# reazon-research/ReazonSpeech

Measured on AMD Instinct MI355X. Metric: RTFx (audio-sec/wall-sec), FastConformer-RNNT 619M batch=256, higher is better.
Workload: dtype bf16

## Files before the change

### reazonspeech_amd/csrc/k_frontend.hip

```cpp
#include "rs_common.h"

namespace {

constexpr int NFFT = 512;
constexpr int NBIN = 257;
constexpr int FB_MAXW = 32;
constexpr int WAVES = 4;
constexpr int FRAMES_PER_WAVE = 4;
constexpr int MAX_HOP = 256;
constexpr int SPAN_MAX = (WAVES * FRAMES_PER_WAVE - 1) * MAX_HOP + NFFT;

struct FrontParams {
    const float* audio; const int32_t* lens; float* raw; int32_t* n_frames;
    const float* window;
    const float* twiddle;
    const int32_t* fb_idx;
    const float* fb_w;
    int audio_stride, pad_left, pad_right, t_max, n_mels, win_length, hop;
    float preemph, log_guard;
    int kind;
};

__device__ __forceinline__ float fetch_sample(const float* __restrict__ a, int i, int pad_left, int len) {
    const int j = i - pad_left;
    return (j >= 0 && j < len) ? a[j] : 0.0f;
}

__device__ __forceinline__ float2 cmul(float2 a, float2 w) { return make_float2(a.x * w.x - a.y * w.y, a.x * w.y + a.y * w.x); }

__device__ __forceinline__ void dft8(float2 (&a)[8]) {
    constexpr float S = 0.70710678118654752f;
    float2 b[8];
#pragma unroll
    for (int j = 0; j < 4; ++j) {
        b[j] = make_float2(a[j].x + a[j + 4].x, a[j].y + a[j + 4].y);
        b[j + 4] = make_float2(a[j].x - a[j + 4].x, a[j].y - a[j + 4].y);
    }
    b[5] = make_float2(S * (b[5].x + b[5].y), S * (b[5].y - b[5].x));
    b[6] = make_float2(b[6].y, -b[6].x);
    b[7] = make_float2(S * (b[7].y - b[7].x), -S * (b[7].x + b[7].y));
    float2 c[8];
#pragma unroll
    for (int h = 0; h < 8; h += 4) {
        c[h + 0] = make_float2(b[h].x + b[h + 2].x, b[h].y + b[h + 2].y);
        c[h + 2] = make_float2(b[h].x - b[h + 2].x, b[h].y - b[h + 2].y);
        c[h + 1] = make_float2(b[h + 1].x + b[h + 3].x, b[h + 1].y + b[h + 3].y);
        const float2 d = make_float2(b[h + 1].x - b[h + 3].x, b[h + 1].y - b[h + 3].y);
        c[h + 3] = make_float2(d.y, -d.x);
    }
    a[0] = make_float2(c[0].x + c[1].x, c[0].y + c[1].y); a[4] = make_float2(c[0].x - c[1].x, c[0].y - c[1].y);
    a[2] = make_float2(c[2].x + c[3].x, c[2].y + c[3].y); a[6] = make_float2(c[2].x - c[3].x, c[2].y - c[3].y);
    a[1] = make_float2(c[4].x + c[5].x, c[4].y + c[5].y); a[5] = make_float2(c[4].x - c[5].x, c[4].y - c[5].y);
    a[3] = make_float2(c[6].x + c[7].x, c[6].y + c[7].y); a[7] = make_float2(c[6].x - c[7].x, c[6].y - c[7].y);
}

__global__ __launch_bounds__(64 * WAVES) void logmel_kernel(FrontParams p) {
    __shared__ float2 buf[WAVES][8 * 68];
    __shared__ float pw[WAVES][2][NBIN + 3];
    __shared__ float2 tw[NFFT / 2];
    __shared__ float ys[SPAN_MAX];
    __shared__ float win_s[NFFT];
    const int lane = threadIdx.x & 63, wave = threadIdx.x >> 6;
    const int b = blockIdx.y;
    const int len = p.lens[b];
    const int Lp = len + p.pad_left + p.pad_right;
    const int n_valid = p.kind == 2 ? (Lp + p.hop / 2) / p.hop
                                    : Lp / p.hop + (p.kind == 1 ? 1 : 0);
    if (blockIdx.x == 0 && threadIdx.x == 0) p.n_frames[b] = n_valid;
    const float* a = p.audio + (size_t)b * p.audio_stride;
    if ((int)blockIdx.x * WAVES * FRAMES_PER_WAVE >= min(n_valid, p.t_max)) return;
    tw[threadIdx.x] = reinterpret_cast<const float2*>(p.twiddle)[threadIdx.x];
    const int centre_off = (NFFT - p.win_length) / 2;
    const int f0 = blockIdx.x * WAVES * FRAMES_PER_WAVE;
    const int i_base = p.kind == 2 ? f0 * p.hop + p.hop / 2 - p.win_length / 2 : f0 * p.hop - NFFT / 2 + centre_off;
    const int span = (WAVES * FRAMES_PER_WAVE - 1) * p.hop + NFFT;
    for (int idx = threadIdx.x; idx < span; idx += blockDim.x) {
        int i = i_base + idx;
        float y = 0.0f;
        if (p.kind == 1 && Lp > 1) {
            i = i < 0 ? -i : i;
            i = i >= Lp ? 2 * (Lp - 1) - i : i;
            i = i < 0 ? 0 : i;
        }
        if (p.kind == 2 && Lp > 0) {
            for (int bounce = 0; bounce < 8 && (i < 0 || i >= Lp); ++bounce) i = i < 0 ? -i - 1 : 2 * Lp - 1 - i;
            i = i < 0 ? 0 : (i >= Lp ? Lp - 1 : i);
        }
        if (i >= 0 && i < Lp) {
            const float x0 = fetch_sample(a, i, p.pad_left, len);
            if (p.kind == 2) y = x0;
            else y = i >= 1 ? x0 - p.preemph * fetch_sample(a, i - 1, p.pad_left, len) : x0;
        }
        ys[idx] = y;
    }
    for (int idx = threadIdx.x; idx < NFFT; idx += blockDim.x) win_s[idx] = idx < p.win_length ? p.window[idx] : 0.0f;
    __syncthreads();
    const int frame_base = (blockIdx.x * WAVES + wave) * FRAMES_PER_WAVE;
    auto wave_sync = [&]() {
        __builtin_amdgcn_fence(__ATOMIC_ACQ_REL, "wavefront");
        __builtin_amdgcn_wave_barrier();
    };
    auto w512 = [&](int j) -> float2 {
        const float2 w = tw[j & 255];
        return (j & 256) ? make_float2(-w.x, -w.y) : w;
    };
    auto sample = [&](int t, int n) -> float {
        if (t >= n_valid || t >= p.t_max) return 0.0f;
        return ys[(t - f0) * p.hop + n] * win_s[n];
    };
    auto frame_mean = [&](int t) -> float {
        if (t >= n_valid || t >= p.t_max) return 0.0f;
        float sm = 0.0f;
        for (int n = lane; n < p.win_length; n += 64) sm += ys[(t - f0) * p.hop + n];
        return wave_sum(sm) / (float)p.win_length;
    };
    auto sample_kaldi = [&](int t, int n, float mean) -> float {
        if (t >= n_valid || t >= p.t_max || n >= p.win_length) return 0.0f;
        const float* fr = ys + (t - f0) * p.hop;
        const float cur = fr[n] - mean, prev = fr[n > 0 ? n - 1 : 0] - mean;
        return (cur - p.preemph * prev) * win_s[n];
    };
    const int k1 = lane & 7, hi = lane >> 3;

    for (int fi = 0; fi < FRAMES_PER_WAVE; fi += 2) {
        const int t = frame_base + fi;
        if (t >= n_valid || t >= p.t_max) break;
        float2* z = buf[wave];
        float2 v[8];
        if (p.kind == 2) {
            const float m0 = frame_mean(t), m1 = frame_mean(t + 1);
#pragma unroll
            for (int k = 0; k < 8; ++k) v[k] = make_float2(sample_kaldi(t, lane + 64 * k, m0), sample_kaldi(t + 1, lane + 64 * k, m1));
        } else {
#pragma unroll
            for (int k = 0; k < 8; ++k) v[k] = make_float2(sample(t, lane + 64 * k), sample(t + 1, lane + 64 * k));
        }
        dft8(v);
#pragma unroll
        for (int q = 0; q < 8; ++q) z[q * 68 + lane] = q ? cmul(v[q], w512(lane * q)) : v[q];
        wave_sync();
#pragma unroll
        for (int l1 = 0; l1 < 8; ++l1) v[l1] = z[k1 * 68 + hi + 8 * l1];
        wave_sync();
        dft8(v);
#pragma unroll
        for (int m1 = 0; m1 < 8; ++m1)
            z[m1 * 64 + ((hi * 8 + k1 + 8 * m1) & 63)] = m1 ? cmul(v[m1], w512(8 * hi * m1)) : v[m1];
        wave_sync();
#pragma unroll
        for (int l2 = 0; l2 < 8; ++l2) v[l2] = z[hi * 64 + ((l2 * 8 + k1 + 8 * hi) & 63)];
        wave_sync();
        dft8(v);
#pragma unroll
        for (int m2 = 0; m2 < 8; ++m2) z[lane + 64 * m2] = v[m2];
        wave_sync();
        for (int k = lane; k < NBIN; k += 64) {
            const float2 zk = z[k], zn = z[(NFFT - k) & (NFFT - 1)];
            const float ar = 0.5f * (zk.x + zn.x), ai = 0.5f * (zk.y - zn.y);
            const float br = 0.5f * (zk.y + zn.y), bi = 0.5f * (zn.x - zk.x);
            pw[wave][0][k] = ar * ar + ai * ai;
            pw[wave][1][k] = br * br + bi * bi;
        }
        wave_sync();
        for (int idx = lane; idx < 2 * p.n_mels; idx += 64) {
            const int f = idx >= p.n_mels, m = idx - f * p.n_mels;
            if (t + f < n_valid && t + f < p.t_max) {
                const int k0 = p.fb_idx[2 * m], cnt = p.fb_idx[2 * m + 1];
                const float* w = p.fb_w + m * FB_MAXW;
                float acc = 0.0f;
                for (int j = 0; j < cnt; ++j) acc = fmaf(w[j], pw[wave][f][k0 + j], acc);
                p.raw[((size_t)b * p.t_max + t + f) * p.n_mels + m] = p.kind >= 1 ? logf(fmaxf(acc, p.log_guard)) : logf(acc + p.log_guard);
            }
        }
        wave_sync();
    }
}

__global__ __launch_bounds__(1024) void feat_normalize_kernel(const float* __restrict__ raw,
                                                              const int32_t* __restrict__ n_frames, int t_max,
                                                              int n_mels, float eps, float* __restrict__ out) {
    __shared__ float4 red[1024];
    __shared__ float4 mean_s[32], rstd_s[32];
    const int b = blockIdx.x;
    const int n = min(n_frames[b], t_max);
    const int Q = n_mels >> 2;
    const int RG = 1000 / Q;
    const int tid = threadIdx.x;
    const int q = tid % Q, rg = tid / Q;
    const bool act = rg < RG;
    const float4* r4 = reinterpret_cast<const float4*>(raw + (size_t)b * t_max * n_mels);
    auto reduce_rows = [&](float4 v) -> float4 {
        red[tid] = act ? v : make_float4(0.f, 0.f, 0.f, 0.f);
        __syncthreads();
        float4 acc = make_float4(0.f, 0.f, 0.f, 0.f);
        if (tid < Q) {
            for (int g = 0; g < RG; ++g) {
                const float4 x = red[g * Q + tid];
                acc.x += x.x; acc.y += x.y; acc.z += x.z; acc.w += x.w;
            }
        }
        return acc;
    };
    float4 s = make_float4(0.f, 0.f, 0.f, 0.f);
    if (act)
#pragma unroll 8
        for (int t = rg; t < n; t += RG) {
            const float4 x = r4[(size_t)t * Q + q];
            s.x += x.x; s.y += x.y; s.z += x.z; s.w += x.w;
        }
    s = reduce_rows(s);
    if (tid < Q) {
        const float inv = 1.0f / (float)n;
        mean_s[tid] = make_float4(s.x * inv, s.y * inv, s.z * inv, s.w * inv);
    }
    __syncthreads();
    const float4 mean = mean_s[q];
    float4 m2 = make_float4(0.f, 0.f, 0.f, 0.f);
    if (act)
#pragma unroll 8
        for (int t = rg; t < n; t += RG) {
            const float4 x = r4[(size_t)t * Q + q];
            const float a = x.x - mean.x, bb = x.y - mean.y, c = x.z - mean.z, d = x.w - mean.w;
            m2.x += a * a; m2.y += bb * bb; m2.z += c * c; m2.w += d * d;
        }
    m2 = reduce_rows(m2);
    if (tid < Q) {
        const float dn = (float)(n - 1);
        rstd_s[tid] = n > 1 ? make_float4(1.0f / (sqrtf(m2.x / dn) + eps), 1.0f / (sqrtf(m2.y / dn) + eps),
                                          1.0f / (sqrtf(m2.z / dn) + eps), 1.0f / (sqrtf(m2.w / dn) + eps))
                            : make_float4(0.f, 0.f, 0.f, 0.f);
    }
    __syncthreads();
    const float4 rstd = rstd_s[q];
    float4* o4 = reinterpret_cast<float4*>(out + (size_t)b * t_max * n_mels);
    if (act)
#pragma unroll 8
        for (int t = rg; t < t_max; t += RG) {
            float4 y = make_float4(0.f, 0.f, 0.f, 0.f);
            if (t < n) {
                const float4 x = r4[(size_t)t * Q + q];
                y = make_float4((x.x - mean.x) * rstd.x, (x.y - mean.y) * rstd.y, (x.z - mean.z) * rstd.z,
                                (x.w - mean.w) * rstd.w);
            }
            o4[(size_t)t * Q + q] = y;
        }
}

__global__ __launch_bounds__(256) void feat_mvn_kernel(const float* __restrict__ raw, const int32_t* __restrict__ n_frames, int t_max,
                                                       int n_mels, const float* __restrict__ mean, const float* __restrict__ istd,
                                                       float* __restrict__ out) {
    const int b = blockIdx.y;
    const int i = blockIdx.x * 256 + threadIdx.x;
    if (i >= t_max * n_mels) return;
    const int t = i / n_mels, m = i - t * n_mels;
    const size_t at = (size_t)b * t_max * n_mels + i;
    out[at] = t < n_frames[b] ? (raw[at] - mean[m]) * istd[m] : 0.0f;
}

}

int rs_launch_frontend(rs_ctx* ctx, const float* audio, const int32_t* lens, int B, int audio_stride,
                       int pad_left, int pad_right, int t_max, float* feats, int32_t* n_frames, float* raw,
                       hipStream_t s) {
    const rs_dims& d = ctx->d;
    if (B <= 0 || t_max <= 0) return RS_OK;
    if (d.n_fft != NFFT) return rs_fail(ctx, RS_EINVAL, "frontend: only n_fft=512 is built");
    if (d.n_mels > 128 || d.n_mels % 4 || d.win_length > NFFT || d.hop_length < 1 || d.hop_length > MAX_HOP)
        return rs_fail(ctx, RS_EINVAL, "frontend: n_mels must be a multiple of 4 up to 128, win <= 512, hop <= %d", MAX_HOP);
    FrontParams p;
    p.audio = audio; p.lens = lens; p.raw = raw; p.n_frames = n_frames;
    p.window = ctx->fe_window; p.twiddle = ctx->fe_twiddle; p.fb_idx = ctx->fe_fb_idx; p.fb_w = ctx->fe_fb_w;
    p.audio_stride = audio_stride; p.pad_left = pad_left; p.pad_right = pad_right; p.t_max = t_max;
    p.n_mels = d.n_mels; p.win_length = d.win_length; p.hop = d.hop_length;
    p.preemph = d.preemph; p.log_guard = d.log_guard;
    p.kind = d.frontend_kind;
    const int fpb = WAVES * FRAMES_PER_WAVE;
    const dim3 grid((t_max + fpb - 1) / fpb, B), block(64 * WAVES);
    if (d.frontend_kind == 2) {
        p.raw = feats;
        RS_HIP(ctx, hipMemsetAsync(feats, 0, (size_t)B * t_max * d.n_mels * 4, s));
    }
    const double bytes = (double)B * ((double)t_max * d.hop_length * 4.0 + (double)t_max * d.n_mels * 4.0 * 3.0);
    rs_prof_begin(ctx, RS_PROF_FRONTEND, s, (double)B * t_max * (5.0 * 512 * 9 + 3 * 257 + 2 * 600), bytes);
    hipLaunchKernelGGL(logmel_kernel, grid, block, 0, s, p);
    if (d.frontend_kind == 2) {
    } else if (d.frontend_kind == 1)
        hipLaunchKernelGGL(feat_mvn_kernel, dim3((t_max * d.n_mels + 255) / 256, B), dim3(256), 0, s, raw, n_frames, t_max, d.n_mels,
                           ctx->fe_mvn_mean, ctx->fe_mvn_istd, feats);
    else
        hipLaunchKernelGGL(feat_normalize_kernel, dim3(B), dim3(1024), 0, s, raw, n_frames, t_max, d.n_mels, d.norm_eps,
                           feats);
    rs_prof_end(ctx, RS_PROF_FRONTEND, s);
    RS_CHECK_LAUNCH(ctx, "frontend");
    return RS_OK;
}
```

### reazonspeech_amd/csrc/rs_api.hip

```cpp
#include <stdarg.h>
#include <stdlib.h>
#include <string.h>

#include <mutex>
#include <set>
#include <utility>

#include "rs_common.h"

size_t rs_rnnt_workspace_bytes(const rs_ctx* ctx, int B);
size_t rs_rnnt_alsd_workspace_bytes_impl(const rs_ctx* ctx, int B, int beam, int cap);
size_t rs_rnnt_beam_workspace_bytes_impl(const rs_ctx* ctx, int B, int beam, int tp_max, int max_pops);
int rs_rnnt_beam_impl(rs_ctx* ctx, const float* joint_enc, const int32_t* enc_lens, int B, int tp_max, int beam, int score_norm,
                      int max_pops, int out_cap, int32_t* ids, int32_t* frames, int32_t* n_ids, float* scores, int32_t* pops,
                      void* workspace, size_t workspace_bytes, hipStream_t s);
int rs_rnnt_alsd_impl(rs_ctx* ctx, const float* joint_enc, const int32_t* enc_lens, int B, int tp_max, int beam, double ratio,
                      int abs_len, int score_norm, int merge, int out_cap, int32_t* ids, int32_t* steps, int32_t* n_ids,
                      float* scores, void* workspace, size_t workspace_bytes, hipStream_t s);
int rs_rnnt_greedy_impl(rs_ctx* ctx, const float* joint_enc, const int32_t* enc_lens, int B, int tp_max, int u_max,
                        int32_t* ids, int32_t* frames, int32_t* n_ids, void* workspace, size_t workspace_bytes,
                        hipStream_t s);

int rs_fail(rs_ctx* ctx, int code, const char* fmt, ...) {
    char buf[512];
// ... 157 lines not shown
    r.get("sub.out.b", dm, ctx->sub_out_b);
    ctx->layers.assign(d.n_layers, rs_layer_w{});
    for (int i = 0; i < d.n_layers; ++i) {
        rs_layer_w& L = ctx->layers[i];
        const std::string p = "L" + std::to_string(i) + ".";
        r.get(p + "ln_ff1.g", dm, L.ln_ff1_g); r.get(p + "ln_ff1.b", dm, L.ln_ff1_b);
        r.get(p + "ff1.w1", ff * dm, L.ff1_w1); r.get(p + "ff1.b1", ff, L.ff1_b1);
        r.get(p + "ff1.w2", dm * ff, L.ff1_w2); r.get(p + "ff1.b2", dm, L.ff1_b2);
        r.get(p + "ln_att.g", dm, L.ln_att_g); r.get(p + "ln_att.b", dm, L.ln_att_b);
        r.get(p + "att.qkv.w", 3 * dm * dm, L.qkv_w); r.get(p + "att.qkv.b", 3 * dm, L.qkv_b);
        r.get(p + "att.out.w", dm * dm, L.out_w); r.get(p + "att.out.b", dm, L.out_b);
        r.get(p + "att.pos.w", dm * dm, L.pos_w);
        r.get(p + "att.bias_u", dm, L.bias_u); r.get(p + "att.bias_v", dm, L.bias_v);
        r.get(p + "ln_conv.g", dm, L.ln_conv_g); r.get(p + "ln_conv.b", dm, L.ln_conv_b);
        r.get(p + "conv.pw1.w", 2 * dm * dm, L.pw1_w); r.get(p + "conv.pw1.b", 2 * dm, L.pw1_b);
        r.get(p + "conv.dw.w", (size_t)d.conv_kernel * dm, L.dw_w); r.get(p + "conv.dw.b", dm, L.dw_b);
        r.get(p + "conv.pw2.w", dm * dm, L.pw2_w); r.get(p + "conv.pw2.b", dm, L.pw2_b);
        r.get(p + "ln_ff2.g", dm, L.ln_ff2_g); r.get(p + "ln_ff2.b", dm, L.ln_ff2_b);
        r.get(p + "ff2.w1", ff * dm, L.ff2_w1); r.get(p + "ff2.b1", ff, L.ff2_b1);
        r.get(p + "ff2.w2", dm * ff, L.ff2_w2); r.get(p + "ff2.b2", dm, L.ff2_b2);
        r.get(p + "ln_out.g", dm, L.ln_out_g); r.get(p + "ln_out.b", dm, L.ln_out_b);
    }
    r.get("joint.enc.w", J * dm, ctx->jenc_w); r.get("joint.enc.b", J, ctx->jenc_b);
    r.get("pred.embed", V * H, ctx->embed);
    for (int l = 0; l < d.pred_layers; ++l) {
        const std::string p = "pred.lstm" + std::to_string(l);
        r.get(p + ".w", 4 * H * 2 * H, ctx->lstm_w[l]);
        r.get(p + ".b", 4 * H, ctx->lstm_b[l]);
    }
    r.get("joint.pred.w", J * H, ctx->jpred_w); r.get("joint.pred.b", J, ctx->jpred_b);
    r.get("joint.out.w", ((V + 15) / 16 * 16) * J, ctx->jout_w); r.get("joint.out.b", V, ctx->jout_b);
    if (r.rc != RS_OK) return r.rc;
    {
        const size_t Vpad = (V + 15) / 16 * 16;
        const bool any = ctx->tensors.count("joint.out.w16") || ctx->tensors.count("joint.out.wrm") ||
                         ctx->tensors.count("joint.out.bpad") || ctx->tensors.count("joint.out.wmax");
        ctx->jout_w16 = nullptr; ctx->jout_wrm = ctx->jout_bpad = ctx->jout_wmax = nullptr;
        if (any) {
            r.get("joint.out.w16", Vpad * J, ctx->jout_w16);
            r.get("joint.out.wrm", V * J, ctx->jout_wrm);
            r.get("joint.out.bpad", Vpad, ctx->jout_bpad);
            r.get("joint.out.wmax", (size_t)4, ctx->jout_wmax);
            if (r.rc != RS_OK) return r.rc;
        }
        for (int l = 0; l < d.pred_layers; ++l) {
            const std::string nm = "pred.lstm" + std::to_string(l) + ".w4";
            ctx->lstm_w4[l] = nullptr;
            if (ctx->tensors.count(nm)) { r.get(nm, 4 * H * 2 * H, ctx->lstm_w4[l]); if (r.rc != RS_OK) return r.rc; }
        }
        if (!ctx->env_read) {
            ctx->env_read = true;
            if (const char* e = getenv("RS_DECODE_SCREEN")) ctx->decode_screen = atoi(e) != 0;
            if (const char* nw = getenv("RS_DECODE_NARROW")) ctx->decode_narrow = atoi(nw) != 0;
            if (const char* fg = getenv("RS_FUSE_GLU")) ctx->fuse_glu = atoi(fg) != 0;
            if (const char* dn = getenv("RS_DEFER_OUT_NORM")) ctx->defer_out_norm = atoi(dn) != 0;
        }
    }
    ctx->has_f32 = false;
    if (ctx->tensors.count("sub.out.w.f32")) {
        rs_f32_weights& w = ctx->f32;
        for (int s = 1; s < d.sub_stages && d.sub_kind == 0; ++s) r.get("sub.pw" + std::to_string(s) + ".w.f32", C * C, w.sub_pw_w[s - 1]);
        if (d.sub_kind == 1) r.get("sub.conv1.w.f32", C * 9 * C, w.sub_conv1_w);
        if (d.ctc_vocab > 0) r.get("ctc.w.f32", (size_t)rs_ctc_pad(d.ctc_vocab) * dm, w.ctc_w);
        r.get("sub.out.w.f32", dm * C * ctx->sub_freq, w.sub_out_w);
        w.layers.assign(d.n_layers, rs_layer_w32{});
        for (int i = 0; i < d.n_layers; ++i) {
            rs_layer_w32& L = w.layers[i];
            const std::string p = "L" + std::to_string(i) + ".";
            r.get(p + "ff1.w1.f32", ff * dm, L.ff1_w1); r.get(p + "ff1.w2.f32", dm * ff, L.ff1_w2);
            r.get(p + "ff2.w1.f32", ff * dm, L.ff2_w1); r.get(p + "ff2.w2.f32", dm * ff, L.ff2_w2);
            r.get(p + "att.qkv.w.f32", 3 * dm * dm, L.qkv_w); r.get(p + "att.out.w.f32", dm * dm, L.out_w);
            r.get(p + "att.pos.w.f32", dm * dm, L.pos_w);
            r.get(p + "conv.pw1.w.f32", 2 * dm * dm, L.pw1_w); r.get(p + "conv.pw1.b.f32", 2 * dm, L.pw1_b);
            r.get(p + "conv.pw2.w.f32", dm * dm, L.pw2_w);
        }
        r.get("joint.enc.w.f32", J * dm, w.jenc_w);
        if (r.rc != RS_OK) return r.rc;
        auto pt = ctx->tensors.find("pos.table.f32");
        if (pt == ctx->tensors.end()) return rs_fail(ctx, RS_EMISSING, "weight tensor 'pos.table.f32' was not registered");
        const size_t rowf = dm * sizeof(float);
        if (pt->second.second % rowf || !((pt->second.second / rowf) & 1) || ((uintptr_t)pt->second.first & 15))
            return rs_fail(ctx, RS_EINVAL, "pos.table.f32 must be 16-byte aligned f32 [2*Tcap-1][d_model]");
        w.pos_table = reinterpret_cast<const float*>(pt->second.first);
        w.pos_table_bytes = pt->second.second;
        ctx->has_f32 = true;
    }
    if (ctx->precision_f32 && !ctx->has_f32) ctx->precision_f32 = 0;
    auto it = ctx->tensors.find("pos.table");
    if (it == ctx->tensors.end()) return rs_fail(ctx, RS_EMISSING, "weight tensor 'pos.table' was not registered");
    const size_t rowb = dm * sizeof(uint16_t);
    if (it->second.second % rowb || !((it->second.second / rowb) & 1))
        return rs_fail(ctx, RS_EINVAL, "pos.table must be bf16 [2*Tcap-1][d_model]");
    for (int i = 0; i < d.n_layers; ++i) {
        auto pp = ctx->tensors.find("L" + std::to_string(i) + ".att.pos_proj");
        if (pp == ctx->tensors.end()) { ctx->layers[i].pos_proj = nullptr; continue; }
        if (pp->second.second != it->second.second || ((uintptr_t)pp->second.first & 15))
            return rs_fail(ctx, RS_EINVAL, "L%d.att.pos_proj must be 16-byte aligned and as large as pos.table", i);
        ctx->layers[i].pos_proj = reinterpret_cast<const uint16_t*>(pp->second.first);
    }
    ctx->finalized = true;
    return RS_OK;
}

int rs_stream_create(void** out, int device, const uint32_t* cu_mask, int n_words, int priority) {
    if (!out) return RS_EINVAL;
    *out = nullptr;
    int cur = -1;
    if (hipGetDevice(&cur) != hipSuccess) return RS_EHIP;
    if (cur != device && hipSetDevice(device) != hipSuccess) return RS_EHIP;
    hipStream_t s = nullptr;
    hipError_t e;
    if (cu_mask && n_words > 0) e = hipExtStreamCreateWithCUMask(&s, (uint32_t)n_words, cu_mask);
    else e = hipStreamCreateWithPriority(&s, hipStreamNonBlocking, priority);
    if (cur != device) hipSetDevice(cur);
    if (e != hipSuccess) return RS_EHIP;
    *out = (void*)s;
    return RS_OK;
}

int rs_stream_destroy(void* stream) {
    if (!stream) return RS_OK;
    return hipStreamDestroy((hipStream_t)stream) == hipSuccess ? RS_OK : RS_EHIP;
}

int rs_set_option(rs_ctx* ctx, const char* key, int value) {
    if (!ctx || !key) return RS_EINVAL;
    if (!strcmp(key, "decode_screen")) { ctx->decode_screen = value != 0; return RS_OK; }
    if (!strcmp(key, "decode_narrow")) { ctx->decode_narrow = value != 0; return RS_OK; }
    if (!strcmp(key, "precision_f32")) {
        if (value && !ctx->has_f32)
            return rs_fail(ctx, RS_EMISSING, "precision_f32: the float32 weights (\"*.f32\" tensors) are not registered / rs_finalize has not run");
        ctx->precision_f32 = value != 0;
        return RS_OK;
    }
    if (!strcmp(key, "precision_i8")) {
        if (!ctx->k2) return rs_fail(ctx, RS_EINVAL, "option 'precision_i8' applies to a Zipformer context only");
        if (value && !(ctx->has_f32 && ctx->has_i8))
            return rs_fail(ctx, RS_EMISSING, "precision_i8: the float32 weights (\"*.f32\") and the quantized ones (\"*.i8\") must be registered and rs_finalize run");
        ctx->precision_i8 = value != 0;
        return RS_OK;
    }
    if (!strcmp(key, "gemm_f32_x3")) {
        ctx->gemm_f32_x3 = value != 0;
        return RS_OK;
    }
    if (!strcmp(key, "k2_conv2_fused")) {
        if (!ctx->k2) return rs_fail(ctx, RS_EINVAL, "option 'k2_conv2_fused' applies to a Zipformer context only");
        ctx->k2_conv2_fused = value != 0;
        return RS_OK;
    }
    if (!strcmp(key, "k2_cnx_fused")) {
        if (!ctx->k2) return rs_fail(ctx, RS_EINVAL, "option 'k2_cnx_fused' applies to a Zipformer context only");
        ctx->k2_cnx_fused = value != 0;
        return RS_OK;
    }
    if (ctx->k2) return rs_fail(ctx, RS_EINVAL, "option '%s' does not apply to a Zipformer context", key);
    if (!strcmp(key, "fuse_glu")) {
        if (value < 0 || value > 1) return rs_fail(ctx, RS_EINVAL, "fuse_glu must be 0 or 1");
        ctx->fuse_glu = value;
        return RS_OK;
    }
    if (!strcmp(key, "defer_out_norm")) { ctx->defer_out_norm = value != 0; return RS_OK; }
    return rs_fail(ctx, RS_EINVAL, "unknown option '%s'", key);
}

int rs_encoder_set_taps(rs_ctx* ctx, float* sub_out, float* layer_out, const int32_t* layer_ids, int n_layer_ids) {
    if (!ctx) return RS_EINVAL;
    if (ctx->k2) return rs_fail(ctx, RS_EINVAL, "taps: a Zipformer context takes rs_k2_encoder_set_taps");
    if (n_layer_ids < 0 || (n_layer_ids > 0 && (!layer_out || !layer_ids))) return rs_fail(ctx, RS_EINVAL, "taps: null pointer");
    for (int i = 0; i < n_layer_ids; ++i)
        if (layer_ids[i] < 0 || layer_ids[i] >= ctx->d.n_layers) return rs_fail(ctx, RS_EINVAL, "taps: layer %d out of range", layer_ids[i]);
    ctx->tap_sub = sub_out;
    ctx->tap_layers = n_layer_ids > 0 ? layer_out : nullptr;
    ctx->tap_ids.assign(layer_ids, layer_ids + n_layer_ids);
    return RS_OK;
}

int rs_mel_frames(const rs_ctx* ctx, int n_samples) {
    if (ctx->d.frontend_kind == 2) return (n_samples + ctx->d.hop_length / 2) / ctx->d.hop_length;
    return n_samples / ctx->d.hop_length + (ctx->d.frontend_kind == 1 ? 1 : 0);
}

int rs_enc_frames(const rs_ctx* ctx, int n) {
    if (ctx->k2) return rs_k2_enc_frames_impl(ctx, n);
    for (int s = 0; s < ctx->d.sub_stages; ++s) n = rs_conv_len(n, ctx->d.sub_kind);
    return n;
}

int rs_encoder_set_ctc_out(rs_ctx* ctx, float* probs, float* blank_prob) {
    if (!ctx) return RS_EINVAL;
    if (ctx->k2 && (probs || blank_prob)) return rs_fail(ctx, RS_EINVAL, "a Zipformer context has no CTC head");
    if ((probs || blank_prob) && ctx->d.ctc_vocab <= 0) return rs_fail(ctx, RS_EINVAL, "this model has no CTC head (rs_dims.ctc_vocab)");
    ctx->ctc_probs = probs;
    ctx->ctc_blank = blank_prob;
    return RS_OK;
}

}

namespace {

struct EncPlan {
    int T[5], F[5];
    size_t off_lens, off_sa, off_sb, off_x, off_hn, off_big, off_ctx, off_posp, off_stats, off_col, off_ctc, total;
    int chunk;
    size_t col_bytes = 0;
};

EncPlan plan_encoder(const rs_ctx* ctx, int B, int t_max) {
    const rs_dims& d = ctx->d;
    EncPlan p{};
    p.T[0] = t_max; p.F[0] = d.n_mels;
    for (int s = 1; s <= d.sub_stages; ++s) { p.T[s] = rs_conv_len(p.T[s - 1], d.sub_kind); p.F[s] = rs_conv_len(p.F[s - 1], d.sub_kind); }
    const size_t C = d.sub_channels, dm = d.d_model;
    const size_t Tp = p.T[d.sub_stages] > 0 ? p.T[d.sub_stages] : 1, M = (size_t)B * Tp;
    size_t widest = (size_t)d.ff_dim;
    if (3 * dm > widest) widest = 3 * dm;
    size_t o = 0;
    p.off_lens = o; o += rs_align((size_t)4 * B * 4);
    p.chunk = B;
    p.off_col = 0;
    if (d.sub_kind == 1) {
        const bool gathered = getenv("RS_SUB_IM2COL") != nullptr;
        const size_t per_utt_col = (size_t)(p.T[2] > 0 ? p.T[2] : 1) * p.F[2] * 9 * C * 2;
        const size_t per_utt_sa = (size_t)(p.T[1] > 0 ? p.T[1] : 1) * p.F[1] * C * 2;
        size_t chunk = gathered ? ((size_t)1 << 30) / per_utt_col : ((size_t)1 << 31) / per_utt_sa;
        if (chunk < 1) chunk = 1;
        if (chunk > (size_t)B) chunk = (size_t)B;
        while (chunk > 1 && chunk * (size_t)(p.T[1] > 0 ? p.T[1] : 1) > 65535) --chunk;
        p.chunk = (int)chunk;
        p.off_sa = o; o += rs_align(chunk * per_utt_sa);
        p.off_col = o; o += gathered ? rs_align(chunk * per_utt_col) : 0;
        p.col_bytes = gathered ? chunk * per_utt_col : 0;
        p.off_sb = o; o += rs_align((size_t)B * (p.T[2] > 0 ? p.T[2] : 1) * p.F[2] * C * 2);
    } else {
        const size_t sub_elems = (size_t)B * p.T[2] * p.F[2] * C;
        p.off_sa = o; o += rs_align(sub_elems * 2);
        p.off_sb = o; o += rs_align(sub_elems * 2);
    }
    p.off_x = o; o += rs_align(M * dm * 4);
    p.off_hn = o; o += rs_align(M * dm * 2);
    p.off_big = o; o += rs_align(M * widest * 2);
    p.off_ctx = o; o += rs_align(M * dm * 2);
    p.off_posp = o; o += rs_align((2 * Tp) * dm * 2);
    p.off_stats = o; o += rs_align(M * 2 * 4);
    p.off_ctc = o;
    if (d.ctc_vocab > 0) o += rs_align(M * (size_t)rs_ctc_pad(d.ctc_vocab) * 4);
    p.total = o + 256;
    return p;
}

}

extern "C" {

size_t rs_workspace_bytes(const rs_ctx* ctx, int B, int max_samples) {
    if (!ctx || B <= 0 || max_samples < 0) return 0;
    const int t_max = rs_mel_frames(ctx, max_samples);
    const size_t fe = rs_align((size_t)B * (t_max > 0 ? t_max : 1) * ctx->d.n_mels * 4) + 256;
    if (ctx->k2) {
        const size_t enc2 = rs_k2_workspace_bytes_impl(ctx, B, t_max), dec2 = rs_rnnt_workspace_bytes(ctx, B);
        const size_t m2 = fe > enc2 ? fe : enc2;
        return m2 > dec2 ? m2 : dec2;
    }
    size_t enc = plan_encoder(ctx, B, t_max > 0 ? t_max : 1).total;
    if (ctx->has_f32) {
        const size_t enc32 = rs_encoder_f32_workspace_bytes(ctx, B, t_max > 0 ? t_max : 1);
        if (enc32 > enc) enc = enc32;
    }
    const size_t dec = rs_rnnt_workspace_bytes(ctx, B);
    size_t m = fe > enc ? fe : enc;
    return m > dec ? m : dec;
}

int rs_host_stage_rows(float* dst, size_t dst_pitch, int width, const float* const* rows, const int32_t* lens,
                       int n_rows, int total_rows, int32_t* dst_lens) {
    if (!dst || !dst_lens || n_rows < 0 || total_rows < n_rows || width < 0 || (size_t)width > dst_pitch) return RS_EINVAL;
    if (n_rows > 0 && (!rows || !lens)) return RS_EINVAL;
    for (int b = 0; b < n_rows; ++b) {
        const int n = lens[b];
        if (n < 0 || n > width || (n > 0 && !rows[b])) return RS_EINVAL;
        float* row = dst + (size_t)b * dst_pitch;
        if (n > 0) memcpy(row, rows[b], (size_t)n * sizeof(float));
        if (n < width) memset(row + n, 0, (size_t)(width - n) * sizeof(float));
        dst_lens[b] = n;
    }
    for (int b = n_rows; b < total_rows; ++b) dst_lens[b] = 0;
    return RS_OK;
}

int rs_frontend_logmel(rs_ctx* ctx, const float* audio, const int32_t* lens, int B, int audio_stride,
                       int pad_left, int pad_right, int t_max, float* feats, int32_t* n_frames, void* workspace,
                       size_t workspace_bytes, void* stream) {
    if (!ctx) return RS_EINVAL;
    if (!ctx->finalized) return rs_fail(ctx, RS_ESTATE, "rs_finalize must precede rs_frontend_logmel");
    if (B < 0 || t_max < 0 || pad_left < 0 || pad_right < 0) return rs_fail(ctx, RS_EINVAL, "frontend: negative size");
    if (B == 0 || t_max == 0) return RS_OK;
    if (!audio || !lens || !feats || !n_frames || !workspace) return rs_fail(ctx, RS_EINVAL, "frontend: null pointer");
    const size_t need = (size_t)B * t_max * ctx->d.n_mels * 4;
    if (workspace_bytes < need) return rs_fail(ctx, RS_EWORKSPACE, "frontend: workspace %zu < %zu", workspace_bytes, need);
    return rs_launch_frontend(ctx, audio, lens, B, audio_stride, pad_left, pad_right, t_max, feats, n_frames,
                              reinterpret_cast<float*>(workspace), (hipStream_t)stream);
}

int rs_encoder_forward(rs_ctx* ctx, const float* feats, const int32_t* n_frames, int B, int t_max, float* enc_out,
                       float* joint_enc, int32_t* enc_lens, void* workspace, size_t workspace_bytes, void* stream) {
// ... 325 lines not shown
```

### reazonspeech_amd/csrc/rs_common.h

```cpp
#pragma once
#include <hip/hip_runtime.h>
#include <stdint.h>
#include <stdio.h>
#include <string>
#include <unordered_map>
#include <vector>

#include "../../include/rs_asr.h"

typedef __bf16 bf16x8_t __attribute__((ext_vector_type(8)));
typedef float f32x4_t __attribute__((ext_vector_type(4)));
typedef float f32x16_t __attribute__((ext_vector_type(16)));
typedef unsigned short u16x8_t __attribute__((ext_vector_type(8)));
typedef unsigned short u16x4_t __attribute__((ext_vector_type(4)));

__device__ __forceinline__ float bf16_to_f32(unsigned short v) {
    return __uint_as_float(((unsigned)v) << 16);
}
typedef __bf16 bf16x4_t __attribute__((ext_vector_type(4)));
typedef __bf16 bf16x2_t __attribute__((ext_vector_type(2)));
__device__ __forceinline__ unsigned short f32_to_bf16(float f) {
    return __builtin_bit_cast(unsigned short, (__bf16)f);
}
__device__ __forceinline__ u16x4_t pack_bf16x4(float a, float b, float c, float d) {
    const f32x4_t v = {a, b, c, d};
    return __builtin_bit_cast(u16x4_t, __builtin_convertvector(v, bf16x4_t));
}
__device__ __forceinline__ float round_bf16(float f) { return bf16_to_f32(f32_to_bf16(f)); }

__device__ __forceinline__ float wave_sum(float v) {
#pragma unroll
    for (int off = 32; off > 0; off >>= 1) v += __shfl_xor(v, off, 64);
    return v;
}
__device__ __forceinline__ float wave_max(float v) {
#pragma unroll
    for (int off = 32; off > 0; off >>= 1) v = fmaxf(v, __shfl_xor(v, off, 64));
    return v;
}
__device__ __forceinline__ float sigmoid_f(float x) { return __builtin_amdgcn_rcpf(1.0f + __expf(-x)); }
__device__ __forceinline__ float silu_f(float x) { return x * sigmoid_f(x); }
__device__ __forceinline__ float softplus_f(float x) { return fmaxf(x, 0.0f) + __logf(1.0f + __expf(-fabsf(x))); }
__device__ __forceinline__ float swoosh_l_f(float x) { return softplus_f(x - 4.0f) - 0.08f * x - 0.035f; }
__device__ __forceinline__ float swoosh_r_f(float x) { return softplus_f(x - 1.0f) - 0.08f * x - 0.313261687f; }
__device__ __forceinline__ float softplus_exact(float x) { return x > 20.0f ? x : log1pf(expf(x)); }
__device__ __forceinline__ float swoosh_l_exact(float x) { return softplus_exact(x - 4.0f) - 0.08f * x - 0.035f; }
__device__ __forceinline__ float swoosh_r_exact(float x) { return softplus_exact(x - 1.0f) - 0.08f * x - 0.313261687f; }

struct rs_prof_launch { int32_t M, N, K, flags; double flops; float ms; };
struct rs_prof_slot {
    std::vector<hipEvent_t> ev;
    std::vector<rs_prof_launch> detail;
    size_t read = 0;
    size_t used = 0;
    double flops = 0, bytes = 0;
    double ms_acc = 0;
    int64_t launches = 0;
};

struct rs_layer_w {
    const float *ln_ff1_g, *ln_ff1_b, *ln_att_g, *ln_att_b, *ln_conv_g, *ln_conv_b, *ln_ff2_g, *ln_ff2_b,
        *ln_out_g, *ln_out_b;
    const uint16_t *ff1_w1, *ff1_w2, *ff2_w1, *ff2_w2, *qkv_w, *out_w, *pos_w, *pw1_w, *pw2_w;
    const float *ff1_b1, *ff1_b2, *ff2_b1, *ff2_b2, *qkv_b, *out_b, *bias_u, *bias_v, *pw1_b, *pw2_b;
    const float *dw_w, *dw_b;
    const uint16_t* pos_proj;
};

struct rs_layer_w32 {
    const float *ff1_w1, *ff1_w2, *ff2_w1, *ff2_w2, *qkv_w, *out_w, *pos_w, *pw1_w, *pw2_w;
    const float* pw1_b;
};
struct rs_f32_weights {
    const float* sub_pw_w[4] = {};
    const float* sub_conv1_w = nullptr;
    const float* ctc_w = nullptr;
    const float* sub_out_w = nullptr;
    std::vector<rs_layer_w32> layers;
    const float* jenc_w = nullptr;
    const float* pos_table = nullptr;
    size_t pos_table_bytes = 0;
};

struct rs_k2;
struct rs_avsr;

struct rs_ctx {
    int device = 0;
    rs_k2* k2 = nullptr;
    void (*k2_free)(rs_k2*) = nullptr;
    rs_avsr* avsr = nullptr;
    void (*avsr_free)(rs_avsr*) = nullptr;
    rs_dims d{};
    int head_dim = 0, sub_freq = 0;
    bool finalized = false;
    std::string err;
    std::unordered_map<std::string, std::pair<const void*, size_t>> tensors;
    const float *fe_window = nullptr, *fe_fb_w = nullptr, *fe_twiddle = nullptr;
    const int32_t* fe_fb_idx = nullptr;
    const float *sub_conv0_w = nullptr, *sub_conv0_b = nullptr;
    const float *sub_dw_w[4] = {}, *sub_dw_b[4] = {};
    const uint16_t* sub_pw_w[4] = {};
    const float* sub_pw_b[4] = {};
    const uint16_t* sub_out_w = nullptr;
    const float* sub_out_b = nullptr;
    std::vector<rs_layer_w> layers;
    const float *fe_mvn_mean = nullptr, *fe_mvn_istd = nullptr;
    const uint16_t* sub_conv1_w = nullptr;
    const float* sub_conv1_b = nullptr;
    const float *final_norm_g = nullptr, *final_norm_b = nullptr;
    const uint16_t* ctc_w = nullptr;
    const float* ctc_b = nullptr;
    float *ctc_probs = nullptr, *ctc_blank = nullptr;
    const uint16_t* jenc_w = nullptr;
    const float* jenc_b = nullptr;
    const float* lstm_w4[8] = {};
    const float* k2_conv_w = nullptr;
    const float *embed = nullptr, *lstm_w[8] = {}, *lstm_b[8] = {}, *jpred_w = nullptr, *jpred_b = nullptr,
                *jout_w = nullptr, *jout_b = nullptr;
    const uint16_t* jout_w16 = nullptr;
    const float *jout_wrm = nullptr, *jout_bpad = nullptr, *jout_wmax = nullptr;
    bool decode_screen = true;
    bool decode_narrow = true;
    bool gemm_f32_x3 = false;
    int k2_conv2_fused = -1;
    int k2_cnx_fused = -1;
    int n_cus = 0;
    int defer_out_norm = 1;
    int fuse_glu = 1;
    bool has_f32 = false;
    int precision_f32 = 0;
    bool has_i8 = false;
    int precision_i8 = 0;
    rs_f32_weights f32;
    bool env_read = false;
    float* tap_sub = nullptr;
    float* tap_layers = nullptr;
    std::vector<int> tap_ids;
    std::unordered_map<const void*, void*> wfm;
    void* wfm_scratch = nullptr;
    size_t wfm_scratch_bytes = 0;
    int prof_mask = 0;
    rs_prof_slot prof[8];
    int32_t prof_tag[4] = {0, 0, 0, 0};
};

int rs_ensure_dynamic_lds(rs_ctx* ctx, const void* func, int bytes);

int rs_fail(rs_ctx* ctx, int code, const char* fmt, ...);

#define RS_HIP(ctx, call)                                                              \
    do {                                                                               \
        hipError_t _e = (call);                                                        \
        if (_e != hipSuccess)                                                          \
            return rs_fail((ctx), RS_EHIP, "%s:%d %s -> %s", __FILE__, __LINE__, #call, \
                           hipGetErrorString(_e));                                     \
    } while (0)

#define RS_CHECK_LAUNCH(ctx, what)                                                            \
    do {                                                                                      \
        hipError_t _e = hipGetLastError();                                                    \
        if (_e != hipSuccess)                                                                 \
            return rs_fail((ctx), RS_EHIP, "launch %s failed: %s", (what), hipGetErrorString(_e)); \
    } while (0)

int rs_prof_class_index(int klass);
void rs_prof_begin(rs_ctx* ctx, int klass, hipStream_t s, double flops, double bytes);
void rs_prof_end(rs_ctx* ctx, int klass, hipStream_t s);

static inline size_t rs_align(size_t x, size_t a = 256) { return (x + a - 1) / a * a; }

struct rs_gemm_args {
    const uint16_t* A; int lda;
    const uint16_t* W; int ldw;
    void* out; int ldc;
    int M, N, K, flags;
    const float* bias; float alpha;
    const float* residual;
    const int32_t* mask_lens; int mask_rows_per_step; int mask_steps;
    const float* res_ln_stats; const float* res_ln_g; const float* res_ln_b;
    uint16_t* out_bf16; int ld_bf16;
    int conv_C, conv_T1, conv_F1, conv_T2, conv_F2;
};
int rs_launch_gemm(rs_ctx* ctx, const rs_gemm_args& a, hipStream_t s);
int rs_launch_layernorm(rs_ctx* ctx, const float* x, const float* g, const float* b, int M, int d, float eps,
                        uint16_t* out_bf16, float* out_f32, hipStream_t s);
int rs_launch_layernorm2(rs_ctx* ctx, const float* x, const float* g1, const float* b1, const float* g2, const float* b2,
                         int M, int d, float eps, float* out_f32, uint16_t* out_bf16, float* stats, hipStream_t s);
int rs_launch_attention(rs_ctx* ctx, const uint16_t* qkv, const uint16_t* pos, const float* bias_u,
                        const float* bias_v, const int32_t* lens, int B, int T, uint16_t* out, hipStream_t s);
int rs_launch_glu_dwconv(rs_ctx* ctx, const uint16_t* x, int layout, const float* w, const float* b, const int32_t* lens,
                         int B, int T, int d, int k, uint16_t* out, hipStream_t s);
int rs_launch_frontend(rs_ctx* ctx, const float* audio, const int32_t* lens, int B, int audio_stride,
                       int pad_left, int pad_right, int t_max, float* feats, int32_t* n_frames, float* raw,
                       hipStream_t s);
int rs_launch_sub_conv0_dw1(rs_ctx* ctx, const float* feats, const int32_t* lens_stage, int B, int t_max, int T2,
                            int F2, uint16_t* out, hipStream_t s);
int rs_launch_sub_dw(rs_ctx* ctx, const uint16_t* in, const float* w, const float* b, const int32_t* lens_out,
                     int stage, int B, int t_in, int f_in, int t_out, int f_out, uint16_t* out, hipStream_t s);
int rs_launch_gemm_f32(rs_ctx* ctx, const float* A, int lda, const float* W, int ldw, float* out, int ldc, int M, int N, int K,
                       int flags, const float* bias, float alpha, const float* residual, const int32_t* mask_lens,
                       int mask_rows_per_step, int mask_steps, hipStream_t s);
int rs_launch_conv3x3_f32(rs_ctx* ctx, const float* in, int n_img, int H, int Wd, int C, int OH, int OW, int stride, const float* W, int Cout,
                          const float* bn_scale, const float* bn_shift, const float* residual, const float* prelu, float* out, int one_by_one, hipStream_t s);
int rs_launch_gemm_f32_skinny(rs_ctx* ctx, const float* A, int lda, const float* W, int ldw, float* out, int ldc, int M, int N, int K, int flags,
                              const float* bias, const float* residual, hipStream_t s);
int rs_launch_attention_f32(rs_ctx* ctx, const float* qkv, const float* pos, const float* bias_u, const float* bias_v,
                            const int32_t* lens, int B, int T, float* out, hipStream_t s);
int rs_launch_glu_dwconv_f32(rs_ctx* ctx, const float* x, const float* w, const float* b, const int32_t* lens, int B, int T,
                             int d, int k, float* out, hipStream_t s);
int rs_launch_i8_range(rs_ctx* ctx, const float* A, int lda, const int32_t* lens, int group, int n_groups, int K, float* qp, hipStream_t s);
int rs_launch_gemm_i8q(rs_ctx* ctx, const float* A, int lda, int group, const float* qp, const int8_t* W, int ldw, const int32_t* colsum,
                       const float* wq, float* out, int ldc, int M, int N, int K, int flags, const float* bias, const float* residual, hipStream_t s);
size_t rs_encoder_f32_workspace_bytes(const rs_ctx* ctx, int B, int t_max);
int rs_encoder_forward_f32(rs_ctx* ctx, const float* feats, const int32_t* n_frames, int B, int t_max, float* enc_out,
                           float* joint_enc, int32_t* enc_lens, void* workspace, size_t workspace_bytes, hipStream_t s);
int rs_launch_enc_lens(rs_ctx* ctx, const int32_t* n_frames, int B, int32_t* lens_out, hipStream_t s);
int rs_launch_sub2d_conv0(rs_ctx* ctx, const float* feats, const int32_t* lens1, int b0, int Bc, int t_max, int T1, int F1,
                          uint16_t* out, hipStream_t s);
int rs_launch_im2col3x3s2(rs_ctx* ctx, const uint16_t* in, int Bc, int T1, int F1, int T2, int F2, uint16_t* out, hipStream_t s);
int rs_launch_ctc_softmax(rs_ctx* ctx, float* logits, int M, int V, int ld, int blank, float* blank_out, hipStream_t s);
int rs_launch_sub2d_conv0_f32(rs_ctx* ctx, const float* feats, const int32_t* lens1, int b0, int Bc, int t_max, int T1, int F1,
                              float* out, hipStream_t s);
int rs_launch_im2col3x3s2_f32(rs_ctx* ctx, const float* in, int Bc, int T1, int F1, int T2, int F2, float* out, hipStream_t s);
static inline int rs_ctc_pad(int v) { return (v + 3) / 4 * 4; }
int rs_avsr_finalize_impl(rs_ctx* ctx);
int rs_k2_finalize_impl(rs_ctx* ctx);
int rs_k2_unk_id(const rs_ctx* ctx);
size_t rs_k2_workspace_bytes_impl(const rs_ctx* ctx, int B, int t_max);
int rs_k2_enc_frames_impl(const rs_ctx* ctx, int n_feat);
int rs_k2_encoder_forward_impl(rs_ctx* ctx, const float* feats, const int32_t* n_frames, int B, int t_max, float* enc_out, float* joint_enc,
                               int32_t* enc_lens, void* workspace, size_t workspace_bytes, hipStream_t s);
int rs_launch_dwconv_act(rs_ctx* ctx, const uint16_t* x, const float* w, const float* b, const int32_t* lens, int B, int T, int d, int k,
                         int act, uint16_t* out, hipStream_t s);
static inline int rs_conv_len(int n, int sub_kind) { return sub_kind ? (n >= 3 ? (n - 3) / 2 + 1 : 0) : (n > 0 ? (n + 2 - 3) / 2 + 1 : 0); }
```

Before: 46100.

## Stage audio span, window and filterbank in LDS for log-mel frontend

```diff
diff --git a/reazonspeech_amd/csrc/k_frontend.hip b/reazonspeech_amd/csrc/k_frontend.hip
--- a/reazonspeech_amd/csrc/k_frontend.hip
+++ b/reazonspeech_amd/csrc/k_frontend.hip
@@ -1,3 +1,5 @@
+#include <cstdlib>
+
 #include "rs_common.h"
 
 namespace {
@@ -176,6 +178,159 @@
     }
 }
 
+constexpr int FBW_STRIDE = FB_MAXW + 1;
+
+struct StagedLds {
+    int pw, win, fbw, fbi, ys, total;
+    __host__ __device__ StagedLds(int n_mels, int hop) {
+        pw = WAVES * 8 * 68 * 8;
+        win = pw + WAVES * 2 * (NBIN + 3) * 4;
+        fbw = win + NFFT * 4;
+        fbi = fbw + n_mels * FBW_STRIDE * 4;
+        ys = fbi + n_mels * 2 * 4;
+        total = ys + ((WAVES * FRAMES_PER_WAVE - 1) * hop + NFFT) * 4;
+    }
+};
+
+__global__ __launch_bounds__(64 * WAVES) void logmel_staged_kernel(FrontParams p) {
+    extern __shared__ __attribute__((aligned(16))) unsigned char lds[];
+    const StagedLds L(p.n_mels, p.hop);
+    float2(*buf)[8 * 68] = reinterpret_cast<float2(*)[8 * 68]>(lds);
+    float(*pw)[2][NBIN + 3] = reinterpret_cast<float(*)[2][NBIN + 3]>(lds + L.pw);
+    float* win_s = reinterpret_cast<float*>(lds + L.win);
+    float* fbw_s = reinterpret_cast<float*>(lds + L.fbw);
+    int32_t* fbi_s = reinterpret_cast<int32_t*>(lds + L.fbi);
+    float* ys = reinterpret_cast<float*>(lds + L.ys);
+    const int lane = threadIdx.x & 63, wave = threadIdx.x >> 6;
+    const int b = blockIdx.y;
+    const int len = p.lens[b];
+    const int Lp = len + p.pad_left + p.pad_right;
+    const int n_valid = p.kind == 2 ? (Lp + p.hop / 2) / p.hop
+                                    : Lp / p.hop + (p.kind == 1 ? 1 : 0);
+    if (blockIdx.x == 0 && threadIdx.x == 0) p.n_frames[b] = n_valid;
+    const float* a = p.audio + (size_t)b * p.audio_stride;
+    if ((int)blockIdx.x * WAVES * FRAMES_PER_WAVE >= min(n_valid, p.t_max)) return;
+    const int centre_off = (NFFT - p.win_length) / 2;
+    const int f0 = blockIdx.x * WAVES * FRAMES_PER_WAVE;
+    const int i_base = p.kind == 2 ? f0 * p.hop + p.hop / 2 - p.win_length / 2 : f0 * p.hop - NFFT / 2 + centre_off;
+    const int span = (WAVES * FRAMES_PER_WAVE - 1) * p.hop + NFFT;
+    for (int idx = threadIdx.x; idx < span; idx += blockDim.x) {
+        int i = i_base + idx;
+        float y = 0.0f;
+        if (p.kind == 1 && Lp > 1) {
+            i = i < 0 ? -i : i;
+            i = i >= Lp ? 2 * (Lp - 1) - i : i;
+            i = i < 0 ? 0 : i;
+        }
+        if (p.kind == 2 && Lp > 0) {
+            for (int bounce = 0; bounce < 8 && (i < 0 || i >= Lp); ++bounce) i = i < 0 ? -i - 1 : 2 * Lp - 1 - i;
+            i = i < 0 ? 0 : (i >= Lp ? Lp - 1 : i);
+        }
+        if (i >= 0 && i < Lp) {
+            const float x0 = fetch_sample(a, i, p.pad_left, len);
+            if (p.kind == 2) y = x0;
+            else y = i >= 1 ? x0 - p.preemph * fetch_sample(a, i - 1, p.pad_left, len) : x0;
+        }
+        ys[idx] = y;
+    }
+    for (int idx = threadIdx.x; idx < NFFT; idx += blockDim.x) win_s[idx] = idx < p.win_length ? p.window[idx] : 0.0f;
+    for (int idx = threadIdx.x; idx < p.n_mels * FB_MAXW; idx += blockDim.x)
+        fbw_s[(idx / FB_MAXW) * FBW_STRIDE + idx % FB_MAXW] = p.fb_w[idx];
+    for (int idx = threadIdx.x; idx < 2 * p.n_mels; idx += blockDim.x) fbi_s[idx] = p.fb_idx[idx];
+    const int k1 = lane & 7, hi = lane >> 3;
+    float2 tw1[8], tw2[8];
+    {
+        const float2* twg = reinterpret_cast<const float2*>(p.twiddle);
+        auto w512 = [&](int j) -> float2 {
+            const float2 w = twg[j & 255];
+            return (j & 256) ? make_float2(-w.x, -w.y) : w;
+        };
+#pragma unroll
+        for (int q = 1; q < 8; ++q) { tw1[q] = w512(lane * q); tw2[q] = w512(8 * hi * q); }
+    }
+    __syncthreads();
+    const int frame_base = (blockIdx.x * WAVES + wave) * FRAMES_PER_WAVE;
+    auto wave_sync = [&]() {
+        __builtin_amdgcn_fence(__ATOMIC_ACQ_REL, "wavefront");
+        __builtin_amdgcn_wave_barrier();
+    };
+    auto sample = [&](int t, int n) -> float {
+        if (t >= n_valid || t >= p.t_max) return 0.0f;
+        return ys[(t - f0) * p.hop + n] * win_s[n];
+    };
+    auto frame_mean = [&](int t) -> float {
+        if (t >= n_valid || t >= p.t_max) return 0.0f;
+        float sm = 0.0f;
+        for (int n = lane; n < p.win_length; n += 64) sm += ys[(t - f0) * p.hop + n];
+        return wave_sum(sm) / (float)p.win_length;
+    };
+    auto sample_kaldi = [&](int t, int n, float mean) -> float {
+        if (t >= n_valid || t >= p.t_max || n >= p.win_length) return 0.0f;
+        const float* fr = ys + (t - f0) * p.hop;
+        const float cur = fr[n] - mean, prev = fr[n > 0 ? n - 1 : 0] - mean;
+        return (cur - p.preemph * prev) * win_s[n];
+    };
+
+    for (int fi = 0; fi < FRAMES_PER_WAVE; fi += 2) {
+        const int t = frame_base + fi;
+        if (t >= n_valid || t >= p.t_max) break;
+        float2* z = buf[wave];
+        float2 v[8];
+        if (p.kind == 2) {
+            const float m0 = frame_mean(t), m1 = frame_mean(t + 1);
+#pragma unroll
+            for (int k = 0; k < 8; ++k) v[k] = make_float2(sample_kaldi(t, lane + 64 * k, m0), sample_kaldi(t + 1, lane + 64 * k, m1));
+        } else {
+#pragma unroll
+            for (int k = 0; k < 8; ++k) v[k] = make_float2(sample(t, lane + 64 * k), sample(t + 1, lane + 64 * k));
+        }
+        dft8(v);
+#pragma unroll
+        for (int q = 0; q < 8; ++q) z[q * 68 + lane] = q ? cmul(v[q], tw1[q]) : v[q];
+        wave_sync();
+#pragma unroll
+        for (int l1 = 0; l1 < 8; ++l1) v[l1] = z[k1 * 68 + hi + 8 * l1];
+        wave_sync();
+        dft8(v);
+#pragma unroll
+        for (int m1 = 0; m1 < 8; ++m1)
+            z[m1 * 64 + ((hi * 8 + k1 + 8 * m1) & 63)] = m1 ? cmul(v[m1], tw2[m1]) : v[m1];
+        wave_sync();
+#pragma unroll
+        for (int l2 = 0; l2 < 8; ++l2) v[l2] = z[hi * 64 + ((l2 * 8 + k1 + 8 * hi) & 63)];
+        wave_sync();
+        dft8(v);
+#pragma unroll
+        for (int m2 = 0; m2 < 8; ++m2) z[lane + 64 * m2] = v[m2];
+        wave_sync();
+        for (int k = lane; k < NBIN; k += 64) {
+            const float2 zk = z[k], zn = z[(NFFT - k) & (NFFT - 1)];
+            const float ar = 0.5f * (zk.x + zn.x), ai = 0.5f * (zk.y - zn.y);
+            const float br = 0.5f * (zk.y + zn.y), bi = 0.5f * (zn.x - zk.x);
+            pw[wave][0][k] = ar * ar + ai * ai;
+            pw[wave][1][k] = br * br + bi * bi;
+        }
+        wave_sync();
+        const bool ok1 = t + 1 < n_valid && t + 1 < p.t_max;
+        for (int m = lane; m < p.n_mels; m += 64) {
+            const int k0 = fbi_s[2 * m], cnt = fbi_s[2 * m + 1];
+            const float* w = fbw_s + m * FBW_STRIDE;
+            const float* p0 = pw[wave][0] + k0;
+            const float* p1 = pw[wave][1] + k0;
+            float acc0 = 0.0f, acc1 = 0.0f;
+            for (int j = 0; j < cnt; ++j) {
+                const float wj = w[j];
+                acc0 = fmaf(wj, p0[j], acc0);
+                acc1 = fmaf(wj, p1[j], acc1);
+            }
+            float* o = p.raw + ((size_t)b * p.t_max + t) * p.n_mels + m;
+            o[0] = p.kind >= 1 ? logf(fmaxf(acc0, p.log_guard)) : logf(acc0 + p.log_guard);
+            if (ok1) o[p.n_mels] = p.kind >= 1 ? logf(fmaxf(acc1, p.log_guard)) : logf(acc1 + p.log_guard);
+        }
+        wave_sync();
+    }
+}
+
 __global__ __launch_bounds__(1024) void feat_normalize_kernel(const float* __restrict__ raw,
                                                               const int32_t* __restrict__ n_frames, int t_max,
                                                               int n_mels, float eps, float* __restrict__ out) {
@@ -282,7 +437,12 @@
     }
     const double bytes = (double)B * ((double)t_max * d.hop_length * 4.0 + (double)t_max * d.n_mels * 4.0 * 3.0);
     rs_prof_begin(ctx, RS_PROF_FRONTEND, s, (double)B * t_max * (5.0 * 512 * 9 + 3 * 257 + 2 * 600), bytes);
-    hipLaunchKernelGGL(logmel_kernel, grid, block, 0, s, p);
+    static const bool staged_env = [] { const char* e = getenv("RS_LOGMEL_STAGED"); return e ? atoi(e) != 0 : true; }();
+    if (ctx->logmel_staged < 0 ? staged_env : ctx->logmel_staged != 0) {
+        const StagedLds L(d.n_mels, d.hop_length);
+        hipLaunchKernelGGL(logmel_staged_kernel, grid, block, L.total, s, p);
+    } else
+        hipLaunchKernelGGL(logmel_kernel, grid, block, 0, s, p);
     if (d.frontend_kind == 2) {
     } else if (d.frontend_kind == 1)
         hipLaunchKernelGGL(feat_mvn_kernel, dim3((t_max * d.n_mels + 255) / 256, B), dim3(256), 0, s, raw, n_frames, t_max, d.n_mels,
diff --git a/reazonspeech_amd/csrc/rs_api.hip b/reazonspeech_amd/csrc/rs_api.hip
--- a/reazonspeech_amd/csrc/rs_api.hip
+++ b/reazonspeech_amd/csrc/rs_api.hip
@@ -333,6 +333,10 @@
     if (!strcmp(key, "k2_cnx_fused")) {
         if (!ctx->k2) return rs_fail(ctx, RS_EINVAL, "option 'k2_cnx_fused' applies to a Zipformer context only");
         ctx->k2_cnx_fused = value != 0;
+        return RS_OK;
+    }
+    if (!strcmp(key, "logmel_staged")) {
+        ctx->logmel_staged = value != 0;
         return RS_OK;
     }
     if (ctx->k2) return rs_fail(ctx, RS_EINVAL, "option '%s' does not apply to a Zipformer context", key);
diff --git a/reazonspeech_amd/csrc/rs_common.h b/reazonspeech_amd/csrc/rs_common.h
--- a/reazonspeech_amd/csrc/rs_common.h
+++ b/reazonspeech_amd/csrc/rs_common.h
@@ -125,6 +125,7 @@
     bool gemm_f32_x3 = false;
     int k2_conv2_fused = -1;
     int k2_cnx_fused = -1;
+    int logmel_staged = -1;
     int n_cus = 0;
     int defer_out_norm = 1;
     int fuse_glu = 1;
```

New measurement: 46330, median of 6. No clear change (+0.5%).
